# pratyushkumar211/industrial_nnmpc_2021

Hardware: AMD Instinct MI355X
Metric: condensed-QP solves/sec (CDU offline datagen) (higher is better)
Workload: dtype f64; 1 GPU; cdu_offline_data: synthetic CDU-size plant (n=4480 vars, m=8960 box rows, n_aug=284), 100000 sampled x0 per GPU per step, whole sequences u* written out; batch_per_gpu=100000, total_batch=100000, method=auto, parallelism=dp1 (sharded samples, 1 RCCL gather of the first moves pe...

## Files before the change

### industrial_nnmpc_2021_amd/csrc/qp_asm.h

```cpp
#pragma once
#include <hip/hip_runtime.h>
#include <stdint.h>
#include <type_traits>

#if defined(ASM_WG_TU) && ASM_WG_TU >= 0
#define ASM_OWN_KERNELS 0
#else
#define ASM_OWN_KERNELS 1
#endif

namespace nnmpc {

constexpr int ASM_MLDS = 176;
constexpr int ASM_TS = 16 * 17;
enum { ASM_RUN = 0, ASM_DONE = 1, ASM_FALLBACK = 2, ASM_CERT = 3, ASM_WIDE = 4, ASM_INVALID = 5 };
constexpr int ASM_NBIN = 8;
constexpr int ASM_NREG = 6;
constexpr int ASM_NCNT = 40;
constexpr int ASM_CNT_F32 = 16;
constexpr int ASM_NLIST = 2 * ASM_NBIN;
constexpr int ASM_BIG32 = 256;
constexpr int ASM_CNT_BIG64 = 37;
constexpr int ASM_CNT_BIG32 = 36;
constexpr int ASM_BIG32B = 384;
// ... 75 lines not shown
  int* lrank;
  int* ctot;
  int use_f32;
  int W;
  int* rowprob;
  int wrows;
  unsigned char* wmark;
  const double* xhw;
  int tail_gi;
  int use_wg;
  int refine;
  double refine_tol;
  int refine_later;
  int early64;
  int* wflag;
  double* work;
  double* scratch;
  double* u_out;
  int ldu, nout;
  uint32_t* act_out;
  int* status_out;
  int* iters_out;
  int words;
};

__device__ __forceinline__ size_t tri(int i, int j) { return (size_t)i * (i + 1) / 2 + j; }

#if ASM_OWN_KERNELS
__global__ __launch_bounds__(256) void asm_init_k(AsmDev d, int nrows) {
  const int lane = threadIdx.x & 63;
// ... 1262 lines not shown
    d.rounds[p] = rd;
    if (tot > 0 && d.hi[p] < W) d.hi[p] = W;
    const bool refine_next = d.refine_later && m <= ASM_MLDS;
    if (tot == 0 && !grade64 && !(f32_phase && refine_next)) d.prec[p] = 1;
    if (tot > 0 && tot <= d.early64 && f32_phase && !refine_next) d.prec[p] = 1;
    if (settle_wide) d.state[p] = ASM_WIDE;
    else if (settled) {
      d.state[p] = sure ? ASM_CERT : ASM_DONE;
      if (!sure) atomicAdd(&d.counters[ASM_CNT_DONE], 1);
    } else if (rd >= d.max_rounds) d.state[p] = ASM_FALLBACK;
  }
}
#endif

#if ASM_OWN_KERNELS
__global__ __launch_bounds__(256) void asm_wide_k(AsmDev d, int fused_c0) {
  const int lane = threadIdx.x & 63;
  const int w = blockIdx.x * 4 + (threadIdx.x >> 6);
  if (w >= d.wrows) return;
  const int p = d.rowprob[w];
  if (p < 0) return;
  const size_t o = (size_t)p * d.np, orow = (size_t)w * d.np;
  const size_t onar = (size_t)d.row[p] * d.np;
  const int Wp = min(d.W, d.n);
  const bool fused = fused_c0 >= 0;
  const int rend = fused ? min(fused_c0, d.n) : d.n;
  unsigned char* st = d.st + (size_t)p * d.n;
  const int m = d.mg[p];
  const int* idx = d.idxg + (size_t)p * d.max_active;
  int chg = 0;
  double l1 = 0.0, lmin = 1e300;
  for (int i = lane; i < m; i += 64) {
    const double l = d.lam[orow + idx[i]];
    l1 += fabs(l); lmin = fmin(lmin, fabs(l));
  }
  for (int r = lane; r < rend; r += 64) {
    const int k = r % d.nu;
    const double lb = d.lb[(size_t)p * d.nu + k], ub = d.ub[(size_t)p * d.nu + k];
    const int s = st[r];
    double x;
    if (s == 0) {
      x = d.xunc[o + r] - (r < Wp ? d.xh[onar + r] : d.xhw[orow + r]);
      if (x > ub + d.bound_tol) { st[r] = 1; ++chg; }
      else if (x < lb - d.bound_tol) { st[r] = 2; ++chg; }
    } else x = s == 1 ? ub : lb;
    if (r < d.nout) d.u_out[(size_t)p * d.ldu + r] = x;
  }
  if (fused && lane == 0) { chg += d.wflag[p]; d.wflag[p] = 0; }
  double x1 = 0.0;
  for (int k = lane; k < d.ka; k += 64) x1 += fabs(d.x0[(size_t)p * d.ka + k]);
  for (int off = 32; off > 0; off >>= 1) {
    chg += __shfl_xor(chg, off);
    l1 += __shfl_xor(l1, off); x1 += __shfl_xor(x1, off);
    lmin = fmin(lmin, __shfl_xor(lmin, off));
  }
  const int tot = chg;
  const double QI = d.tqmax * x1;
  const double bnd = 2.0 * (d.e1max * x1 + d.e2max * l1) + 1e-14 * (QI + l1) + d.ff_err * (x1 + l1);
  const bool sure = bnd <= d.stat_tol * d.pscale && lmin > bnd;
  if (tot == 0 && !sure) {
    for (int r = lane; r < d.n; r += 64) {
      const int k = r % d.nu, s = st[r];
      double x;
      if (s != 0) x = s == 1 ? d.ub[(size_t)p * d.nu + k] : d.lb[(size_t)p * d.nu + k];
      else if (r < Wp) x = d.xunc[o + r] - d.xh[onar + r];
      else if (!fused) x = d.xunc[o + r] - d.xhw[orow + r];
      else {
        const double* Hc = d.H + r;
        double a0 = 0.0;
        for (int i = 0; i < m; ++i) { const int a = idx[i]; a0 += Hc[(size_t)a * d.np] * d.lam[orow + a]; }
        double xu;
        if (r < d.Wx) xu = d.xunc[o + r];
        else {
          xu = 0.0;
          for (int k2 = 0; k2 < d.ka; ++k2) xu += d.Kunc[(size_t)r * d.ka + k2] * d.x0[(size_t)p * d.ka + k2];
        }
        x = xu - a0;
      }
      d.x[o + r] = x;
    }
  }
  for (int i = lane; i < m; i += 64) d.lam[orow + idx[i]] = 0.0;
  if (lane == 0) {
    d.wmark[p] = 1;
    if (tot == 0) {
      d.state[p] = sure ? ASM_CERT : ASM_DONE;
      if (!sure) atomicAdd(&d.counters[ASM_CNT_DONE], 1);
    } else {
      d.state[p] = d.rounds[p] >= d.max_rounds ? ASM_FALLBACK : ASM_RUN;
      d.ninf_best[p] = 0x7fffffff; d.alpha[p] = ASM_GRACE;
      d.hi[p] = d.n;
    }
  }
}
#endif

constexpr int ASM_FM = 160;
constexpr int ASM_TAIL_GRACE = 2;
constexpr int ASM_TAIL_AREA = ASM_FM * (ASM_FM + 3) / 2 > ASM_TAIL_MB * (ASM_TAIL_MB + 1) / 2 * ASM_TS
                                  ? ASM_FM * (ASM_FM + 3) / 2 : ASM_TAIL_MB * (ASM_TAIL_MB + 1) / 2 * ASM_TS;
constexpr int ASM_TAIL_EXTRA = ASM_FM * (4 + 8 + 8 + 8);
__device__ __forceinline__ int asm_frow(int i) { return i * (i + 3) / 2; }

static_assert(ASM_FM <= 192, "asm_fwd / asm_bwd hold the vector in at most three registers per lane");
template <int NU>
__device__ __forceinline__ void asm_fwd_t(const double* Ld, double* v, int m, int lane) {
  double x[NU], idg[NU], ln[NU];
  const double* rowp[NU];
// ... 446 lines not shown
            --mm;
          }
        }
        if (lane == 0) { s_m = mm; s_fast = ok; }
      }
      __syncthreads();
      m = s_m; fast = s_fast;
    }
    __syncthreads();
  }
  if (tid == 0) { d.state[p] = ASM_FALLBACK; d.rounds[p] = rounds; }
}
#endif

#if ASM_OWN_KERNELS
__global__ __launch_bounds__(256) void asm_certify_k(AsmDev d, double gscale_min) {
  __shared__ int cnt[4];
  __shared__ double gq[4];
  const int p = blockIdx.x, tid = threadIdx.x;
  const int stt = d.state[p];
  if (stt == ASM_INVALID) {
    const double qnan = __longlong_as_double(0x7ff8000000000000ll);
    for (int r = tid; r < d.nout; r += 256) d.u_out[(size_t)p * d.ldu + r] = qnan;
    if (d.act_out) for (int w = tid; w < d.words; w += 256) d.act_out[(size_t)p * d.words + w] = 0u;
    if (tid == 0) {
      if (d.status_out) d.status_out[p] = 2;
      if (d.iters_out) { d.iters_out[2 * p] = 0; d.iters_out[2 * p + 1] = 0; }
    }
    return;
  }
  if (stt != ASM_DONE && stt != ASM_CERT) {
    if (tid == 0 && d.status_out) d.status_out[p] = 3;
    return;
  }
// ... 41 lines not shown
          const int kk = r / d.nu, c = r - kk * d.nu;
          const int bit = kk * 2 * d.nu + (sv == 1 ? c : d.nu + c), w = (bit >> 5) - w0;
          if (w >= 0 && w < nwd) atomicOr(&wb[w], 1u << (bit & 31));
        }
      }
      __syncthreads();
      for (int w = tid; w < nwd; w += 256) d.act_out[(size_t)p * d.words + w0 + w] = wb[w];
      __syncthreads();
    }
  }
  if (tid == 0) {
    if (d.status_out) d.status_out[p] = ok ? 0 : 3;
    if (d.iters_out) { d.iters_out[2 * p] = 0; d.iters_out[2 * p + 1] = 0; }
  }
}
#endif

#if ASM_OWN_KERNELS
__global__ void asm_gather_k(double* x0c, double* lbc, double* ubc, const double* x0, const double* lb,
                             const double* ub, const int* list, int cnt, int n_aug, int nu) {
  const int i = blockIdx.x;
  if (i >= cnt) return;
  const int p = list[i];
  for (int k = threadIdx.x; k < n_aug; k += blockDim.x) x0c[(size_t)i * n_aug + k] = x0[(size_t)p * n_aug + k];
  for (int k = threadIdx.x; k < nu; k += blockDim.x) {
    lbc[(size_t)i * nu + k] = lb[(size_t)p * nu + k];
    ubc[(size_t)i * nu + k] = ub[(size_t)p * nu + k];
  }
}
#endif
// ... 27 lines not shown
```

### industrial_nnmpc_2021_amd/csrc/qp_solver.hip

```cpp
#include <hip/hip_runtime.h>
#include <stdint.h>
#include <stdio.h>
#include <stdarg.h>
#include <string.h>
#include <vector>
#include <algorithm>
#include <cmath>
#include <cstdlib>
#include "../../include/nnmpc.h"
#define ASM_WG_TU (-1)
#include "chol_kernels.h"
#include "gemm_kernels.h"
#include "qp_asm.h"
#include "qp_wide.h"
#include "qp_small.h"
#include "qp_predict.h"
#include "common.h"
static constexpr int ASM_SMALL9_LDS_MAX = 100 * 1024;

using namespace nnmpc;

namespace {

enum { PH_INIT = 0, PH_IPM = 1, PH_POLISH = 2, PH_DONE = 3 };
// ... 588 lines not shown
  double* P64;
  double* tq64;
  float* Kunc32;
  float* pdiag;
  double pscale;
  float* L;
  float* Y;
  float* Dacc;
  unsigned long long* trsv_count;
  QpDev d;
  bool have_inverse;
  double* H64;
  double* Kunc64;
  double *asm_xunc, *asm_x, *asm_lam, *asm_xh, *asm_scratch, *asm_xhw;
  int *asm_rowprob, *asm_wflag;
  unsigned char* asm_wmark;
  unsigned char* asm_st;
  int *asm_state, *asm_rounds, *asm_counters, *asm_biglist, *asm_status, *asm_binlist, *asm_idxg, *asm_mg, *asm_row, *asm_lrank, *asm_ctot;
  unsigned char *asm_prec, *asm_redo, *asm_alpha, *asm_rowk;
  float *asm_lam32, *asm_xh32, *H32;
  int *asm_ninf, *asm_hi, *asm_kblk;
  double tqmax;
  int asm_pool;
  double asm_e1max, asm_e2max;
  struct Far { int W, r, rp; double *U, *Vx, *Vl, *cu; int* kt; double ksum; double efar; };
  std::vector<Far> far;
  std::vector<int> far_missing;
  double p_inf = 0.0;
  double *asm_tnorm = nullptr, *asm_tslack = nullptr;
  struct AsmView {
    double *lam = nullptr, *xh = nullptr, *xhw = nullptr, *tnorm = nullptr, *tslack = nullptr;
// ... 7 lines not shown
  int* pred_cnt = nullptr;
  double* asm_work;
  int seg_max;
  double* x0_64;
  float* x0_32;
  double* q64_all;
  float* uunc_all;
  double *lb_d, *ub_d;
  double* in_stage;
  hipStream_t stream;
  hipStream_t stream2 = nullptr;
  hipStream_t stream3 = nullptr, stream4 = nullptr;
  int asm_tail_budget = 50000;
  hipEvent_t ev_fork = nullptr, ev_join = nullptr, ev_join3 = nullptr, ev_join4 = nullptr;
  hipEvent_t ev_wfork = nullptr, ev_wide = nullptr;
  int* pin_cnt = nullptr;
  int* pin_st = nullptr;
  bool profiling;
  bool gemm_error = false;
  std::vector<hipEvent_t> ev_pool;
  size_t ev_used;
  struct EvRec { int kind; size_t e0, e1; double flops; };
  std::vector<EvRec> ev_recs;
  nnmpc_qp_stats stats;
  std::vector<void*> allocs;
  struct Scratch { void* p = nullptr; size_t cap = 0; };
  enum { SC_U = 0, SC_ACT, SC_ST, SC_IT, SC_GUESS, SC_FB_GUESS, SC_FB_LIST, SC_FB_X0, SC_FB_LB, SC_FB_UB, SC_FB_U, SC_FB_ACT, SC_FB_ST, SC_FB_IT, SC_COUNT };
  Scratch sc[SC_COUNT];
  int ldu, nout;
};
// ... 274 lines not shown
    EvScope es(h, 5, 2.0 * Wx * (double)h->ka * nprob);
    gemm64(h, h->asm_xunc, h->np, h->x0_64, h->ka, h->Kunc64, h->ka, segp, Wx, h->ka);
  }
  AsmDev a;
  a.Kunc = h->Kunc64; a.Wx = Wx; a.winit = winit;
  a.ffU = a.ffVx = a.ffVl = a.ffcu = nullptr; a.ffk = nullptr; a.ffr = a.ffW = 0; a.T = h->asm_xhw; a.tnorm = h->asm_tnorm; a.tslack = h->asm_tslack;
  a.ff_skip = 0; a.ff_err = 0.0; a.ff_efar = 0.0;
  static const bool no_far = getenv("NNMPC_NO_FARFIELD") != nullptr;
  a.n = h->n; a.np = h->np; a.nu = h->nu; a.nseg = nprob;
  a.max_active = h->opts.asm_max_active; a.max_rounds = h->opts.asm_max_rounds;
  a.bound_tol = h->opts.bound_tol; a.stat_tol = 1e-8; a.pscale = h->pscale;
  a.e1max = h->asm_e1max; a.e2max = h->asm_e2max; a.x0 = h->x0_64; a.ka = h->ka;
  a.H = h->H64; a.lb = lb_dev; a.ub = ub_dev; a.xunc = h->asm_xunc; a.q64 = h->q64_all;
  a.x = h->asm_x; a.lam = h->asm_lam; a.xh = h->asm_xh; a.px = h->asm_xh;
  a.st = h->asm_st; a.guess = guess_dev; a.state = h->asm_state; a.rounds = h->asm_rounds; a.counters = h->asm_counters;
  a.biglist = h->asm_biglist; a.binlist = h->asm_binlist; a.idxg = h->asm_idxg; a.mg = h->asm_mg; a.row = h->asm_row; a.tqmax = h->tqmax; a.lrank = h->asm_lrank; a.ctot = h->asm_ctot; a.prec = h->asm_prec; a.redo = h->asm_redo; a.rowk = h->asm_rowk; a.lam32 = h->asm_lam32; a.H32 = h->H32; a.xh32 = h->asm_xh32; a.alpha = h->asm_alpha; a.ninf_best = h->asm_ninf; a.hi = h->asm_hi; a.kblk = h->asm_kblk; a.nkblk = 2 * (h->seg_max / 64 + 2); a.kref = 0; a.use_f32 = h->opts.asm_f32_rounds >= 0; a.xhw = h->asm_xhw; a.rowprob = h->asm_rowprob; a.wrows = 0; a.wmark = h->asm_wmark; a.wflag = h->asm_wflag; a.W = h->np; a.scratch = h->asm_scratch; a.work = h->asm_work;
  a.u_out = u_dev; a.ldu = h->ldu; a.nout = h->nout; a.act_out = act_dev; a.status_out = h->asm_status; a.iters_out = it_dev; a.words = h->words;
  a.nseg = nprob;
  { static const int tgi = getenv("NNMPC_TAIL_GI") ? 1 : 0; a.tail_gi = tgi; }
  { static const int wg = getenv("NNMPC_NO_WG") ? 0 : 1; a.use_wg = wg; }
  { static const int rfn = getenv("NNMPC_REFINE") ? atoi(getenv("NNMPC_REFINE")) : 1; a.refine = 0; a.refine_later = rfn && a.use_f32;
    static const double rtol = getenv("NNMPC_REFINE_TOL") ? atof(getenv("NNMPC_REFINE_TOL")) : ASM_REFINE_TOL; a.refine_tol = rtol; }
  { static const int e64 = getenv("NNMPC_EARLY64") ? atoi(getenv("NNMPC_EARLY64")) : 4; a.early64 = e64; }
  if (!guess_dev) HIPCHK(hipMemsetAsync(h->asm_st, 0, (size_t)nprob * h->n, s));
  a.pred_w = 0; a.pred_f64 = 0;
  double pred_flops_per_it = 0.0;
  {
    static const int env_it = getenv("NNMPC_PRED_ITERS") ? atoi(getenv("NNMPC_PRED_ITERS")) : -1;
    const int iters_req = env_it >= 0 ? (env_it == 0 ? -1 : std::min(env_it, (int)PRED_MAXIT)) : h->opts.asm_predict_iters;
    const int iters = iters_req == 0 ? (int)PRED_MAXIT : iters_req;
    if (iters > 0 && h->pred[0].L > 0.0 && !guess_dev && !small && !tail_only && Wx >= PRED_W) {
// ... 29 lines not shown
      h->stats.asm_predict_launches += 1;
      EvScope es(h, 10, 0.0);
      if (wide) hipLaunchKernelGGL((asm_predict_k<8, 2>), dim3((nprob + 31) / 32), dim3(64 * PRED_NW), (pred_lds_bytes<8, 2>(h->nu)), s, a, pa);
      else if (nu4) hipLaunchKernelGGL((asm_predict_k<4, 4>), dim3((nprob + 63) / 64), dim3(64 * PRED_NW), (pred_lds_bytes<4, 4>(h->nu)), s, a, pa);
      else hipLaunchKernelGGL((asm_predict_k<4, 2, false>), dim3((nprob + 31) / 32), dim3(64 * PRED_NW), (pred_lds_bytes<4, 2>(h->nu)), s, a, pa);
      a.pred_w = W;
      { static const int pf = getenv("NNMPC_PRED_F64") ? atoi(getenv("NNMPC_PRED_F64")) : 0; a.pred_f64 = pf; }
    }
  }
  hipLaunchKernelGGL(asm_init_k, dim3((segp + 3) / 4), dim3(256), 0, s, a, segp);
  const int lds_big = (a.max_active + ASM_TS) * 8;
  int* cnt = h->pin_cnt;
  memset(cnt, 0, 2 * ASM_NCNT * sizeof(int));
  int rounds = 0;
  int kprev = 0;
  HIPCHK(hipMemsetAsync(h->asm_counters, 0, 2 * ASM_NCNT * sizeof(int), s));
  if (small) {
    EvScope es(h, 4, 0.0);
    static const int g0 = getenv("NNMPC_SMALL_GRACE") ? atoi(getenv("NNMPC_SMALL_GRACE")) : ASM_SM_GRACE;
    hipLaunchKernelGGL((asm_small_k<2, 3, 4>), dim3(nprob), dim3(64), asm_small_lds_bytes(2, h->n, h->nu), s, a, a.max_rounds, g0);
    hipLaunchKernelGGL((asm_small_k<7, 1, 8>), dim3(nprob), dim3(64), asm_small_lds_bytes(7, h->n, h->nu), s, a, a.max_rounds, g0);
    if (asm_small_lds_bytes(9, h->n, h->nu) <= ASM_SMALL9_LDS_MAX)
      hipLaunchKernelGGL((asm_small_k<9, 1, 8>), dim3(nprob), dim3(64), asm_small_lds_bytes(9, h->n, h->nu), s, a, a.max_rounds, g0);
    h->stats.asm_rounds += 1;
    h->stats.asm_small_passes += 1;
    static const bool trace = getenv("NNMPC_TRACE_ROUNDS") != nullptr;
    if (trace) {
      std::vector<int> rd(nprob), mg(nprob), stt(nprob);
      HIPCHK(stream_sync(s));
      hipMemcpy(rd.data(), h->asm_rounds, nprob * sizeof(int), hipMemcpyDeviceToHost);
      hipMemcpy(mg.data(), h->asm_mg, nprob * sizeof(int), hipMemcpyDeviceToHost);
// ... 33 lines not shown
      std::vector<int> rd(nprob), mg(nprob);
      hipMemcpy(rd.data(), h->asm_rounds, nprob * sizeof(int), hipMemcpyDeviceToHost);
      hipMemcpy(mg.data(), h->asm_mg, nprob * sizeof(int), hipMemcpyDeviceToHost);
      long sum = 0, sm = 0; int mx = 0, mm = 0;
      for (int i = 0; i < nprob; ++i) { sum += rd[i]; mx = std::max(mx, rd[i]); sm += mg[i]; mm = std::max(mm, mg[i]); }
      fprintf(stderr, "asm tail only: %d problems, iterations mean %.2f max %d, active bounds mean %.1f max %d\n", nprob, (double)sum / nprob, mx, (double)sm / nprob, mm);
    }
  }
  auto set_view = [&](AsmDev& d, int v) {
    const nnmpc_qp::AsmView& V = h->view[v];
    d.lam = V.lam; d.xh = V.xh; d.xhw = V.xhw; d.T = V.xhw; d.tnorm = V.tnorm; d.tslack = V.tslack; d.lam32 = V.lam32; d.xh32 = V.xh32;
    d.rowprob = V.rowprob; d.kblk = V.kblk; d.counters = V.counters;
  };
  const char* env_ovl = getenv("NNMPC_OVERLAP");
  const bool overlap_on = h->opts.asm_overlap >= 0 && h->view[1].rows > 0 && !(env_ovl && atoi(env_ovl) == 0);
  int vW[2] = {h->np, h->np}, vrows[2] = {0, 0};
  int pend = -1;
  bool tail_ran[2] = {false, false};
  struct WideStat { bool open; int view, far_rp, skip, cols; double far_ksum; } wst = {false, 0, 0, 0, 0, 0.0}, wnext = wst;
  int fft_prev[2] = {0, 0};
  auto account = [&](const int* c) {
    if (!wst.open) return;
    wst.open = false;
    if (!h->profiling) return;
    const double nw = c[ASM_CNT_WIDE + 1], ksum = c[ASM_CNT_WKSUM];
    if (wst.far_rp) {
      const int fft = h->pin_cnt[wst.view * ASM_NCNT + ASM_CNT_FFTILES];
      const double chunks = fft - fft_prev[wst.view];
      fft_prev[wst.view] = fft;
      h->stats.asm_gemm_flops += 2.0 * wst.far_rp * (ksum + nw * h->ka) +
// ... 36 lines not shown
        HIPCHK(hipStreamWaitEvent(ps, h->ev_wfork, 0));
      }
      ap.ff_err = 0.0; ap.ff_efar = 0.0; ap.ff_skip = 0;
      int far_rp = 0;
      double far_ksum = 0.0;
      {
        EvScope es(h, 5, 0.0, ps);
        if (ff) {
          ap.ffU = ff->U; ap.ffVx = ff->Vx; ap.ffVl = ff->Vl; ap.ffcu = ff->cu; ap.ffk = ff->kt; ap.ffr = ff->rp; ap.ffW = ff->W;
          ap.ff_err = h->p_inf * ff->efar; ap.ff_efar = ff->efar;
          ap.ff_skip = h->nout <= c0 && h->nout < h->n;
          far_rp = ff->rp; far_ksum = ff->ksum;
          h->stats.asm_far_passes += 1;
          hipLaunchKernelGGL(asm_wide_t_k, dim3(g64_grid(ntm, ff->rp / 128)), dim3(256), G64_LDS, ps, ap, ntm, ff->rp / 128);
          if (ap.ff_skip) hipLaunchKernelGGL(asm_wide_tnorm_k, dim3((ntm * 128 + 3) / 4), dim3(256), 0, ps, ap, ntm);
          hipLaunchKernelGGL(asm_wide_gemm_k<WIDE_FAR>, dim3(g64_grid(ntm, ntn)), dim3(256), G64_LDS, ps, ap, c0, ntm, ntn);
        } else if (fused_c0 >= 0 && lazy) {
          hipLaunchKernelGGL(asm_wide_gemm_k<WIDE_LAZY>, dim3(g64_grid(ntm, ntn)), dim3(256), G64_LDS, s, ap, c0, ntm, ntn);
        } else if (fused_c0 >= 0) {
          hipLaunchKernelGGL(asm_wide_gemm_k<WIDE_XUNC>, dim3(g64_grid(ntm, ntn)), dim3(256), G64_LDS, s, ap, c0, ntm, ntn);
        } else {
          gemm64(h, h->view[pv].xhw + c0, h->np, h->view[pv].lam, h->np, h->H64 + (size_t)c0 * h->np, h->np, ((prev_rows + 127) / 128) * 128,
                 h->np - c0, h->np, nullptr, 0, h->view[pv].kblk, nullptr, true);
        }
      }
      wnext.view = pv; wnext.far_rp = far_rp; wnext.far_ksum = far_ksum; wnext.skip = ap.ff_skip; wnext.cols = h->np - c0; wnext.open = true;
      if (ovl) {
        HIPCHK(hipEventRecord(h->ev_wide, ps));
        inflight = true;
      } else {
        EvScope es(h, 6, 0.0);
        hipLaunchKernelGGL(asm_wide_k, dim3((prev_rows + 3) / 4), dim3(256), 0, s, ap, fused_c0);
        wst = wnext;
      }
      pend = -1; vrows[pv] = 0;
    }
    auto finish_pass = [&]() -> int {
      HIPCHK(hipStreamWaitEvent(s, h->ev_wide, 0));
      EvScope es(h, 6, 0.0);
      hipLaunchKernelGGL(asm_wide_k, dim3((ap.wrows + 3) / 4), dim3(256), 0, s, ap, fused_c0);
      wst = wnext;
      inflight = false;
      return 0;
    };
    if (!a.pred_w) a.refine_later = 0;
    a.refine = a.refine_later && rounds >= 1;
    a.kref = kprev;
    int rv = inflight ? 1 - pv : 0;
    int n64 = 0, n32 = 0, nrun = 0;
    for (;;) {
      set_view(a, rv);
      cnt = h->pin_cnt + rv * ASM_NCNT;
      {
        EvScope es(h, 6, 0.0);
        hipLaunchKernelGGL(asm_count_k, dim3((nprob + 3) / 4), dim3(256), 0, s, a);
// ... 158 lines not shown
    }
  }
  if (rounds >= 2 * a.max_rounds + 2) {
    HIPCHK(hipMemcpyAsync(h->pin_cnt, h->asm_counters, 2 * ASM_NCNT * sizeof(int), hipMemcpyDeviceToHost, s));
    HIPCHK(stream_sync(s));
  }
  if (h->gemm_error) { h->gemm_error = false; return NNMPC_EINVAL; }
  set_view(a, 0);
  cnt = h->pin_cnt;
  auto ndone = [&]() { return h->pin_cnt[ASM_CNT_DONE] + h->pin_cnt[ASM_NCNT + ASM_CNT_DONE]; };
  if (!defer_cnt) h->stats.asm_full_checks += ndone();
  if (defer_cnt || ndone() > 0) {
    gemm64(h, h->q64_all, h->np, h->x0_64, h->ka, h->tq64, h->ka, segp, h->np, h->ka, h->asm_state, ASM_DONE);
    gemm64(h, h->asm_xh, h->np, h->asm_x, h->np, h->P64, h->np, segp, h->np, h->np, h->asm_state, ASM_DONE);
  }
  hipLaunchKernelGGL(asm_certify_k, dim3(nprob), dim3(256), 0, s, a, h->pscale);
  int* st = h->pin_st;
  HIPCHK(hipMemcpyAsync(st, h->asm_status, (size_t)nprob * sizeof(int), hipMemcpyDeviceToHost, s));
  int* pin_its = h->pin_cnt + 2 * ASM_NCNT;
  if (h->profiling && pred_flops_per_it > 0.0) HIPCHK(hipMemcpyAsync(pin_its, h->pred_cnt + 1, 4, hipMemcpyDeviceToHost, s));
  if (defer_cnt) HIPCHK(hipMemcpyAsync(h->pin_cnt, h->asm_counters, 2 * ASM_NCNT * sizeof(int), hipMemcpyDeviceToHost, s));
  HIPCHK(stream_sync(s));
  if (defer_cnt) h->stats.asm_full_checks += ndone();
  if (h->profiling && pred_flops_per_it > 0.0) h->stats.asm_predict_flops += pred_flops_per_it * (double)*pin_its;
  HIPCHK(hipGetLastError());
  std::vector<int> fb;
  int ninvalid = 0;
  for (int p = 0; p < nprob; ++p) { if (st[p] == 3) fb.push_back(p); else if (st[p] != 0) ++ninvalid; }
  h->stats.asm_solved += nprob - (int64_t)fb.size() - ninvalid;
  if (st_dev) HIPCHK(hipMemcpyAsync(st_dev, h->asm_status, (size_t)nprob * sizeof(int), hipMemcpyDeviceToDevice, s));
  if (fb.empty()) { h->stats.problems += nprob; return 0; }
// ... 86 lines not shown
  h->n = n; h->nu = nu; h->n_aug = n_aug;
  h->NB = o.nb;
  h->np = ((n + h->NB - 1) / h->NB) * h->NB;
  h->T = h->np / h->NB;
  h->tiles = h->T * (h->T + 1) / 2;
  h->ka = ((n_aug + 31) / 32) * 32;
  h->slots = ((o.max_batch + 127) / 128) * 128;
  h->words = (2 * n + 31) / 32;
  h->have_kunc = Kunc != nullptr;
  if ((size_t)(h->np + 5 * h->NB) * 4 > 96 * 1024) { set_error("n too large for the LDS-resident solve vector"); delete h; return NNMPC_EINVAL; }
  if (hipStreamCreate(&h->stream) != hipSuccess) { set_error("hipStreamCreate failed"); delete h; return NNMPC_EHIP; }
  if (hipStreamCreate(&h->stream2) != hipSuccess || hipStreamCreate(&h->stream3) != hipSuccess || hipStreamCreate(&h->stream4) != hipSuccess ||
      hipEventCreateWithFlags(&h->ev_fork, hipEventDisableTiming) != hipSuccess ||
      hipEventCreateWithFlags(&h->ev_join3, hipEventDisableTiming) != hipSuccess || hipEventCreateWithFlags(&h->ev_join4, hipEventDisableTiming) != hipSuccess ||
      hipEventCreateWithFlags(&h->ev_join, hipEventDisableTiming) != hipSuccess ||
      hipEventCreateWithFlags(&h->ev_wfork, hipEventDisableTiming) != hipSuccess || hipEventCreateWithFlags(&h->ev_wide, hipEventDisableTiming) != hipSuccess) {
    set_error("hipStreamCreate / hipEventCreate failed"); nnmpc_qp_destroy(h); return NNMPC_EHIP;
  }
  {
    hipError_t e = hipSuccess;
    if (e == hipSuccess) e = hipFuncSetAttribute((const void*)asm_lambda_reg_k, hipFuncAttributeMaxDynamicSharedMemorySize, ASM_REG_LDS);
    if (e == hipSuccess) e = hipFuncSetAttribute((const void*)asm_lambda_reg2_k, hipFuncAttributeMaxDynamicSharedMemorySize, ASM_REG2_LDS);
    if (e == hipSuccess) e = hipFuncSetAttribute((const void*)asm_lambda_reg32_k, hipFuncAttributeMaxDynamicSharedMemorySize, ASM_REG32_LDS);
    if (e == hipSuccess) e = hipFuncSetAttribute((const void*)asm_tail_k, hipFuncAttributeMaxDynamicSharedMemorySize, 150 * 1024);
    if (e == hipSuccess) e = hipFuncSetAttribute((const void*)asm_lambda_reg32b_k, hipFuncAttributeMaxDynamicSharedMemorySize, ASM_REG32B_LDS);
    if (e == hipSuccess) e = hipFuncSetAttribute((const void*)asm_lambda_tile32_k, hipFuncAttributeMaxDynamicSharedMemorySize, ASM_TILE32_LDS);
    if (e == hipSuccess) e = hipFuncSetAttribute((const void*)gemm_nt_f64_t128_k, hipFuncAttributeMaxDynamicSharedMemorySize, G64_LDS);
    if (e == hipSuccess) e = hipFuncSetAttribute((const void*)asm_wide_gemm_k<WIDE_XUNC>, hipFuncAttributeMaxDynamicSharedMemorySize, G64_LDS);
    if (e == hipSuccess) e = hipFuncSetAttribute((const void*)asm_wide_gemm_k<WIDE_LAZY>, hipFuncAttributeMaxDynamicSharedMemorySize, G64_LDS);
    if (e == hipSuccess) e = hipFuncSetAttribute((const void*)asm_wide_gemm_k<WIDE_FAR>, hipFuncAttributeMaxDynamicSharedMemorySize, G64_LDS);
    if (e == hipSuccess) e = hipFuncSetAttribute((const void*)asm_wide_t_k, hipFuncAttributeMaxDynamicSharedMemorySize, G64_LDS);
// ... 29 lines not shown
    cap = std::min<long long>(cap, 1 << 20);
    h->seg_max = (int)((cap / 128) * 128);
  }
  const size_t G = h->seg_max;
  A_(h->x0_64, G * ka); A_(h->x0_32, G * ka);
  A_(h->q64_all, G * np); A_(h->uunc_all, G * np);
  A_(h->lb_d, G * nu); A_(h->ub_d, G * nu);
  A_(h->in_stage, G * n_aug);
  if (!rc && hipHostMalloc((void**)&h->pin_cnt, (2 * ASM_NCNT + 4) * sizeof(int)) != hipSuccess) { set_error("nnmpc_qp_create: hipHostMalloc failed"); rc = NNMPC_EHIP; }
  if (!rc && hipHostMalloc((void**)&h->pin_st, G * sizeof(int)) != hipSuccess) { set_error("nnmpc_qp_create: hipHostMalloc failed"); rc = NNMPC_EHIP; }
  A_(d.lb64, (size_t)S * nu); A_(d.ub64, (size_t)S * nu);
  A_(d.slot_prob, S); A_(d.age, S); A_(d.next_prob, 1);
  h->asm_pool = h->seg_max >= 4096 ? (getenv("NNMPC_TAIL_MAX") && atoi(getenv("NNMPC_TAIL_MAX")) > 1024 ? 2048 : 1024) : 256;
  A_(h->H64, (size_t)np * np); A_(h->Kunc64, (size_t)np * ka); A_(h->H32, (size_t)np * np);
  A_(h->asm_xunc, G * np); A_(h->asm_x, G * np); A_(h->asm_lam, G * np); A_(h->asm_xh, G * np);
  A_(h->asm_xhw, (G + 256) * np); A_(h->asm_rowprob, G + 256); A_(h->asm_wflag, G); A_(h->asm_wmark, G);
  A_(h->asm_tnorm, G + 128 * (ASM_NKG + 1)); A_(h->asm_tslack, G + 128 * (ASM_NKG + 1));
  A_(h->asm_st, G * n); A_(h->asm_state, G); A_(h->asm_rounds, G); A_(h->asm_counters, 2 * ASM_NCNT);
  A_(h->asm_biglist, G); A_(h->asm_status, G); A_(h->asm_binlist, (size_t)(ASM_NLIST + 4) * G);
  A_(h->asm_idxg, G * o.asm_max_active); A_(h->asm_mg, G); A_(h->asm_row, G); A_(h->asm_lrank, G); A_(h->asm_ctot, ((G + 1023) / 1024) * ASM_NSCAN); A_(h->asm_prec, G); A_(h->asm_redo, G); A_(h->asm_rowk, G); A_(h->asm_lam32, G * np); A_(h->asm_xh32, G * np); A_(h->asm_alpha, G); A_(h->asm_ninf, G); A_(h->asm_hi, G); A_(h->asm_kblk, 2 * (G / 64 + 2)); A_(h->asm_work, 3 * G);
  A_(h->asm_scratch, (size_t)h->asm_pool * ((size_t)(o.asm_max_active / 16) * (o.asm_max_active / 16 + 1) / 2 * ASM_TS));
  {
    nnmpc_qp::AsmView& v0 = h->view[0];
    v0.lam = h->asm_lam; v0.xh = h->asm_xh; v0.xhw = h->asm_xhw; v0.tnorm = h->asm_tnorm; v0.tslack = h->asm_tslack;
    v0.lam32 = h->asm_lam32; v0.xh32 = h->asm_xh32; v0.rowprob = h->asm_rowprob; v0.kblk = h->asm_kblk; v0.counters = h->asm_counters;
    v0.rows = (int)G;
    long long R = std::max<long long>(1024, ((long long)G / 32 + 127) / 128 * 128);
    if (const char* e = getenv("NNMPC_OVERLAP_ROWS")) R = std::max(0, atoi(e) / 128 * 128);
    R = std::min<long long>(R, (long long)G);
    if (o.asm_overlap >= 0 && R > 0) {
      nnmpc_qp::AsmView& v1 = h->view[1];
      const size_t Rr = (size_t)R;
      A_(v1.lam, Rr * np); A_(v1.xh, Rr * np); A_(v1.xhw, (Rr + 256) * np); A_(v1.lam32, Rr * np); A_(v1.xh32, Rr * np);
// ... 69 lines not shown
}

int nnmpc_qp_destroy(nnmpc_qp* h) {
  if (!h) return NNMPC_OK;
  hipDeviceSynchronize();
  for (void* p : h->allocs) hipFree(p);
  for (auto& g : h->far) { hipFree(g.U); hipFree(g.Vx); hipFree(g.Vl); hipFree(g.cu); hipFree(g.kt); }
  for (auto& sc : h->sc) if (sc.p) hipFree(sc.p);
  for (hipEvent_t e : h->ev_pool) hipEventDestroy(e);
  if (h->ev_fork) hipEventDestroy(h->ev_fork);
  if (h->ev_join) hipEventDestroy(h->ev_join);
  if (h->ev_join3) hipEventDestroy(h->ev_join3);
  if (h->ev_join4) hipEventDestroy(h->ev_join4);
  if (h->ev_wfork) hipEventDestroy(h->ev_wfork);
  if (h->ev_wide) hipEventDestroy(h->ev_wide);
  if (h->pin_cnt) hipHostFree(h->pin_cnt);
  if (h->pin_st) hipHostFree(h->pin_st);
  if (h->stream2) hipStreamDestroy(h->stream2);
  if (h->stream3) hipStreamDestroy(h->stream3);
  if (h->stream4) hipStreamDestroy(h->stream4);
  if (h->stream) hipStreamDestroy(h->stream);
  delete h;
  return NNMPC_OK;
}

int nnmpc_qp_set_inverse(nnmpc_qp* h, const double* Hinv, const double* Kunc) {
  if (!h || !Hinv || !Kunc) { set_error("nnmpc_qp_set_inverse: bad arguments"); return NNMPC_EINVAL; }
  HIPCHK(hipSetDevice(h->device));
  const int n = h->n, np = h->np, ka = h->ka, n_aug = h->n_aug;
  if ((uint64_t)np * np * 8 >= (1ull << 32)) {
// ... 300 lines not shown
```

Baseline: 7.635 million solves/s.

## Split wide-pass finish to overlap with far GEMM; wave-per-problem certify kernel

The wide-pass epilogue is split in two. A pre-kernel does the bound check and certificate test as soon as the lambda-dependent work is recorded, overlapping the far-side wide GEMM on the side stream. A decision kernel then finishes after the GEMM completes. Certification now runs one wave per problem for certified, invalid and other-state cases, compacting DONE problems into a list that a block-per-problem kernel processes. The goal is to hide wide-pass latency and cut idle blocks in certify, at the cost of extra launches, events and an atomic list counter.

```diff
diff --git a/industrial_nnmpc_2021_amd/csrc/qp_asm.h b/industrial_nnmpc_2021_amd/csrc/qp_asm.h
--- a/industrial_nnmpc_2021_amd/csrc/qp_asm.h
+++ b/industrial_nnmpc_2021_amd/csrc/qp_asm.h
@@ -113,6 +113,8 @@
   int refine_later;
   int early64;
   int* wflag;
+  unsigned char* wpre;
+  int* certn;
   double* work;
   double* scratch;
   double* u_out;
@@ -1405,50 +1407,12 @@
 #endif
 
 #if ASM_OWN_KERNELS
-__global__ __launch_bounds__(256) void asm_wide_k(AsmDev d, int fused_c0) {
-  const int lane = threadIdx.x & 63;
-  const int w = blockIdx.x * 4 + (threadIdx.x >> 6);
-  if (w >= d.wrows) return;
-  const int p = d.rowprob[w];
-  if (p < 0) return;
-  const size_t o = (size_t)p * d.np, orow = (size_t)w * d.np;
-  const size_t onar = (size_t)d.row[p] * d.np;
+__device__ __forceinline__ void asm_wide_finish(const AsmDev& d, int p, int w, int lane, bool fused, int tot, bool sure, bool zero_lam) {
+  const size_t o = (size_t)p * d.np, orow = (size_t)w * d.np, onar = (size_t)d.row[p] * d.np;
   const int Wp = min(d.W, d.n);
-  const bool fused = fused_c0 >= 0;
-  const int rend = fused ? min(fused_c0, d.n) : d.n;
-  unsigned char* st = d.st + (size_t)p * d.n;
+  const unsigned char* st = d.st + (size_t)p * d.n;
   const int m = d.mg[p];
   const int* idx = d.idxg + (size_t)p * d.max_active;
-  int chg = 0;
-  double l1 = 0.0, lmin = 1e300;
-  for (int i = lane; i < m; i += 64) {
-    const double l = d.lam[orow + idx[i]];
-    l1 += fabs(l); lmin = fmin(lmin, fabs(l));
-  }
-  for (int r = lane; r < rend; r += 64) {
-    const int k = r % d.nu;
-    const double lb = d.lb[(size_t)p * d.nu + k], ub = d.ub[(size_t)p * d.nu + k];
-    const int s = st[r];
-    double x;
-    if (s == 0) {
-      x = d.xunc[o + r] - (r < Wp ? d.xh[onar + r] : d.xhw[orow + r]);
-      if (x > ub + d.bound_tol) { st[r] = 1; ++chg; }
-      else if (x < lb - d.bound_tol) { st[r] = 2; ++chg; }
-    } else x = s == 1 ? ub : lb;
-    if (r < d.nout) d.u_out[(size_t)p * d.ldu + r] = x;
-  }
-  if (fused && lane == 0) { chg += d.wflag[p]; d.wflag[p] = 0; }
-  double x1 = 0.0;
-  for (int k = lane; k < d.ka; k += 64) x1 += fabs(d.x0[(size_t)p * d.ka + k]);
-  for (int off = 32; off > 0; off >>= 1) {
-    chg += __shfl_xor(chg, off);
-    l1 += __shfl_xor(l1, off); x1 += __shfl_xor(x1, off);
-    lmin = fmin(lmin, __shfl_xor(lmin, off));
-  }
-  const int tot = chg;
-  const double QI = d.tqmax * x1;
-  const double bnd = 2.0 * (d.e1max * x1 + d.e2max * l1) + 1e-14 * (QI + l1) + d.ff_err * (x1 + l1);
-  const bool sure = bnd <= d.stat_tol * d.pscale && lmin > bnd;
   if (tot == 0 && !sure) {
     for (int r = lane; r < d.n; r += 64) {
       const int k = r % d.nu, s = st[r];
@@ -1471,7 +1435,7 @@
       d.x[o + r] = x;
     }
   }
-  for (int i = lane; i < m; i += 64) d.lam[orow + idx[i]] = 0.0;
+  if (zero_lam) for (int i = lane; i < m; i += 64) d.lam[orow + idx[i]] = 0.0;
   if (lane == 0) {
     d.wmark[p] = 1;
     if (tot == 0) {
@@ -1483,6 +1447,90 @@
       d.hi[p] = d.n;
     }
   }
+}
+#endif
+
+#if ASM_OWN_KERNELS
+__device__ __forceinline__ int asm_wide_window(const AsmDev& d, int p, int w, int lane, int rend, bool& sure) {
+  const size_t o = (size_t)p * d.np, orow = (size_t)w * d.np;
+  const size_t onar = (size_t)d.row[p] * d.np;
+  const int Wp = min(d.W, d.n);
+  unsigned char* st = d.st + (size_t)p * d.n;
+  const int m = d.mg[p];
+  const int* idx = d.idxg + (size_t)p * d.max_active;
+  int chg = 0;
+  double l1 = 0.0, lmin = 1e300;
+  for (int i = lane; i < m; i += 64) {
+    const double l = d.lam[orow + idx[i]];
+    l1 += fabs(l); lmin = fmin(lmin, fabs(l));
+  }
+  for (int r = lane; r < rend; r += 64) {
+    const int k = r % d.nu;
+    const double lb = d.lb[(size_t)p * d.nu + k], ub = d.ub[(size_t)p * d.nu + k];
+    const int s = st[r];
+    double x;
+    if (s == 0) {
+      x = d.xunc[o + r] - (r < Wp ? d.xh[onar + r] : d.xhw[orow + r]);
+      if (x > ub + d.bound_tol) { st[r] = 1; ++chg; }
+      else if (x < lb - d.bound_tol) { st[r] = 2; ++chg; }
+    } else x = s == 1 ? ub : lb;
+    if (r < d.nout) d.u_out[(size_t)p * d.ldu + r] = x;
+  }
+  double x1 = 0.0;
+  for (int k = lane; k < d.ka; k += 64) x1 += fabs(d.x0[(size_t)p * d.ka + k]);
+  for (int off = 32; off > 0; off >>= 1) {
+    chg += __shfl_xor(chg, off);
+    l1 += __shfl_xor(l1, off); x1 += __shfl_xor(x1, off);
+    lmin = fmin(lmin, __shfl_xor(lmin, off));
+  }
+  const double QI = d.tqmax * x1;
+  const double bnd = 2.0 * (d.e1max * x1 + d.e2max * l1) + 1e-14 * (QI + l1) + d.ff_err * (x1 + l1);
+  sure = bnd <= d.stat_tol * d.pscale && lmin > bnd;
+  return chg;
+}
+#endif
+
+#if ASM_OWN_KERNELS
+__global__ __launch_bounds__(256) void asm_wide_k(AsmDev d, int fused_c0) {
+  const int lane = threadIdx.x & 63;
+  const int w = blockIdx.x * 4 + (threadIdx.x >> 6);
+  if (w >= d.wrows) return;
+  const int p = d.rowprob[w];
+  if (p < 0) return;
+  const bool fused = fused_c0 >= 0;
+  bool sure;
+  int tot = asm_wide_window(d, p, w, lane, fused ? min(fused_c0, d.n) : d.n, sure);
+  if (fused) { tot += d.wflag[p]; if (lane == 0) d.wflag[p] = 0; }
+  asm_wide_finish(d, p, w, lane, fused, tot, sure, true);
+}
+
+__global__ __launch_bounds__(256) void asm_wide_pre_k(AsmDev d, int fused_c0) {
+  const int lane = threadIdx.x & 63;
+  const int w = blockIdx.x * 4 + (threadIdx.x >> 6);
+  if (w >= d.wrows) return;
+  const int p = d.rowprob[w];
+  if (p < 0) return;
+  bool sure;
+  const int chg = asm_wide_window(d, p, w, lane, min(fused_c0, d.n), sure);
+  if (sure) {
+    const size_t orow = (size_t)w * d.np;
+    const int m = d.mg[p];
+    const int* idx = d.idxg + (size_t)p * d.max_active;
+    for (int i = lane; i < m; i += 64) d.lam[orow + idx[i]] = 0.0;
+  }
+  if (lane == 0) d.wpre[p] = (unsigned char)((sure ? 1 : 0) | (chg > 0 ? 2 : 0));
+}
+__global__ __launch_bounds__(256) void asm_wide_dec_k(AsmDev d) {
+  const int lane = threadIdx.x & 63;
+  const int w = blockIdx.x * 4 + (threadIdx.x >> 6);
+  if (w >= d.wrows) return;
+  const int p = d.rowprob[w];
+  if (p < 0) return;
+  const int pre = d.wpre[p];
+  const bool sure = (pre & 1) != 0;
+  const int tot = (pre >> 1) + d.wflag[p];
+  if (lane == 0) d.wflag[p] = 0;
+  asm_wide_finish(d, p, w, lane, true, tot, sure, !sure);
 }
 #endif
 
@@ -1959,10 +2007,10 @@
 #endif
 
 #if ASM_OWN_KERNELS
-__global__ __launch_bounds__(256) void asm_certify_k(AsmDev d, double gscale_min) {
+__device__ __forceinline__ void asm_certify_one(const AsmDev& d, double gscale_min, int p) {
   __shared__ int cnt[4];
   __shared__ double gq[4];
-  const int p = blockIdx.x, tid = threadIdx.x;
+  const int tid = threadIdx.x;
   const int stt = d.state[p];
   if (stt == ASM_INVALID) {
     const double qnan = __longlong_as_double(0x7ff8000000000000ll);
@@ -2034,6 +2082,106 @@
     if (d.iters_out) { d.iters_out[2 * p] = 0; d.iters_out[2 * p + 1] = 0; }
   }
 }
+__global__ __launch_bounds__(256) void asm_certify_k(AsmDev d, double gscale_min) { asm_certify_one(d, gscale_min, blockIdx.x); }
+
+__global__ __launch_bounds__(256) void asm_certify_list_k(AsmDev d, double gscale_min) {
+  const int nl = *d.certn;
+  for (int i = blockIdx.x; i < nl; i += gridDim.x) {
+    asm_certify_one(d, gscale_min, d.biglist[i]);
+    __syncthreads();
+  }
+}
+
+__global__ __launch_bounds__(256) void asm_certify_wave_k(AsmDev d, double gscale_min) {
+  __shared__ uint32_t wbs[4][256];
+  const int lane = threadIdx.x & 63, wv = threadIdx.x >> 6;
+  const int p = blockIdx.x * 4 + wv;
+  if (p >= d.nseg) return;
+  const int stt = d.state[p];
+  if (stt == ASM_DONE) {
+    if (lane == 0) d.biglist[atomicAdd(d.certn, 1)] = p;
+    return;
+  }
+  if (stt == ASM_INVALID) {
+    const double qnan = __longlong_as_double(0x7ff8000000000000ll);
+    for (int r = lane; r < d.nout; r += 64) d.u_out[(size_t)p * d.ldu + r] = qnan;
+    if (d.act_out) for (int w = lane; w < d.words; w += 64) d.act_out[(size_t)p * d.words + w] = 0u;
+    if (lane == 0) {
+      if (d.status_out) d.status_out[p] = 2;
+      if (d.iters_out) { d.iters_out[2 * p] = 0; d.iters_out[2 * p + 1] = 0; }
+    }
+    return;
+  }
+  if (stt != ASM_CERT) {
+    if (lane == 0 && d.status_out) d.status_out[p] = 3;
+    return;
+  }
+  const int ok = 0.0 <= d.stat_tol * fmax(gscale_min, 0.0);
+  if (d.act_out) {
+    uint32_t* ao = d.act_out + (size_t)p * d.words;
+    const unsigned char* st = d.st + (size_t)p * d.n;
+    const int nu = d.nu;
+    const int rlim = min((min(d.hi[p], d.n) + nu - 1) / nu * nu, d.n);
+    const bool whole = d.n % nu == 0;
+    if (whole && nu < 32 && 32 % nu == 0) {
+      const uint32_t msk = (1u << nu) - 1u;
+      for (int r0 = 0; r0 < rlim; r0 += 64) {
+        const int r = r0 + lane;
+        const int sv = r < rlim ? st[r] : 0;
+        const unsigned long long U = __ballot(sv == 1), L = __ballot(sv == 2);
+        const int w = (r0 >> 4) + lane;
+        if (lane < 4 && w < d.words) {
+          const uint32_t u16 = (uint32_t)(U >> (16 * lane)) & 0xffffu, l16 = (uint32_t)(L >> (16 * lane)) & 0xffffu;
+          uint32_t word = 0u;
+          for (int g = 0; g * nu < 16; ++g)
+            word |= (((u16 >> (g * nu)) & msk) << (2 * g * nu)) | (((l16 >> (g * nu)) & msk) << (2 * g * nu + nu));
+          ao[w] = word;
+        }
+      }
+      for (int w = min(d.words, (rlim + 63) / 64 * 4) + lane; w < d.words; w += 64) ao[w] = 0u;
+    } else if (whole && nu % 32 == 0) {
+      const int cps = nu / 32;
+      for (int r0 = 0; r0 < rlim; r0 += 64) {
+        const int r = r0 + lane;
+        const int sv = r < rlim ? st[r] : 0;
+        const unsigned long long U = __ballot(sv == 1), L = __ballot(sv == 2);
+        const int j = (r0 >> 5) + (lane >> 1);
+        if (lane < 4 && 32 * j < rlim) {
+          const int kk = j / cps, cj = j - kk * cps;
+          ao[kk * 2 * cps + (lane & 1) * cps + cj] = (uint32_t)(((lane & 1) ? L : U) >> (32 * (lane >> 1)));
+        }
+      }
+      for (int w = rlim / nu * 2 * cps + lane; w < d.words; w += 64) ao[w] = 0u;
+    } else {
+      uint32_t* wb = wbs[wv];
+      for (int w0 = 0; w0 < d.words; w0 += 256) {
+        const int nwd = min(256, d.words - w0);
+        const int k0 = (32 * w0) / (2 * nu), k1 = min(rlim / nu + (rlim % nu != 0), (32 * (w0 + nwd) + 2 * nu - 1) / (2 * nu));
+        if (k0 * nu >= rlim) {
+          for (int w = lane; w < nwd; w += 64) ao[w0 + w] = 0u;
+          continue;
+        }
+        for (int w = lane; w < nwd; w += 64) wb[w] = 0u;
+        ASM_FENCE();
+        for (int r = k0 * nu + lane; r < min(k1 * nu, rlim); r += 64) {
+          const int sv = st[r];
+          if (sv) {
+            const int kk = r / nu, c = r - kk * nu;
+            const int bit = kk * 2 * nu + (sv == 1 ? c : nu + c), w = (bit >> 5) - w0;
+            if (w >= 0 && w < nwd) atomicOr(&wb[w], 1u << (bit & 31));
+          }
+        }
+        ASM_FENCE();
+        for (int w = lane; w < nwd; w += 64) ao[w0 + w] = wb[w];
+        ASM_FENCE();
+      }
+    }
+  }
+  if (lane == 0) {
+    if (d.status_out) d.status_out[p] = ok ? 0 : 3;
+    if (d.iters_out) { d.iters_out[2 * p] = 0; d.iters_out[2 * p + 1] = 0; }
+  }
+}
 #endif
 
 #if ASM_OWN_KERNELS
diff --git a/industrial_nnmpc_2021_amd/csrc/qp_solver.hip b/industrial_nnmpc_2021_amd/csrc/qp_solver.hip
--- a/industrial_nnmpc_2021_amd/csrc/qp_solver.hip
+++ b/industrial_nnmpc_2021_amd/csrc/qp_solver.hip
@@ -626,7 +626,7 @@
   double* Kunc64;
   double *asm_xunc, *asm_x, *asm_lam, *asm_xh, *asm_scratch, *asm_xhw;
   int *asm_rowprob, *asm_wflag;
-  unsigned char* asm_wmark;
+  unsigned char *asm_wmark, *asm_wpre;
   unsigned char* asm_st;
   int *asm_state, *asm_rounds, *asm_counters, *asm_biglist, *asm_status, *asm_binlist, *asm_idxg, *asm_mg, *asm_row, *asm_lrank, *asm_ctot;
   unsigned char *asm_prec, *asm_redo, *asm_alpha, *asm_rowk;
@@ -664,6 +664,7 @@
   int asm_tail_budget = 50000;
   hipEvent_t ev_fork = nullptr, ev_join = nullptr, ev_join3 = nullptr, ev_join4 = nullptr;
   hipEvent_t ev_wfork = nullptr, ev_wide = nullptr;
+  hipEvent_t ev_wlam = nullptr;
   int* pin_cnt = nullptr;
   int* pin_st = nullptr;
   bool profiling;
@@ -968,7 +969,7 @@
   a.H = h->H64; a.lb = lb_dev; a.ub = ub_dev; a.xunc = h->asm_xunc; a.q64 = h->q64_all;
   a.x = h->asm_x; a.lam = h->asm_lam; a.xh = h->asm_xh; a.px = h->asm_xh;
   a.st = h->asm_st; a.guess = guess_dev; a.state = h->asm_state; a.rounds = h->asm_rounds; a.counters = h->asm_counters;
-  a.biglist = h->asm_biglist; a.binlist = h->asm_binlist; a.idxg = h->asm_idxg; a.mg = h->asm_mg; a.row = h->asm_row; a.tqmax = h->tqmax; a.lrank = h->asm_lrank; a.ctot = h->asm_ctot; a.prec = h->asm_prec; a.redo = h->asm_redo; a.rowk = h->asm_rowk; a.lam32 = h->asm_lam32; a.H32 = h->H32; a.xh32 = h->asm_xh32; a.alpha = h->asm_alpha; a.ninf_best = h->asm_ninf; a.hi = h->asm_hi; a.kblk = h->asm_kblk; a.nkblk = 2 * (h->seg_max / 64 + 2); a.kref = 0; a.use_f32 = h->opts.asm_f32_rounds >= 0; a.xhw = h->asm_xhw; a.rowprob = h->asm_rowprob; a.wrows = 0; a.wmark = h->asm_wmark; a.wflag = h->asm_wflag; a.W = h->np; a.scratch = h->asm_scratch; a.work = h->asm_work;
+  a.biglist = h->asm_biglist; a.binlist = h->asm_binlist; a.idxg = h->asm_idxg; a.mg = h->asm_mg; a.row = h->asm_row; a.tqmax = h->tqmax; a.lrank = h->asm_lrank; a.ctot = h->asm_ctot; a.prec = h->asm_prec; a.redo = h->asm_redo; a.rowk = h->asm_rowk; a.lam32 = h->asm_lam32; a.H32 = h->H32; a.xh32 = h->asm_xh32; a.alpha = h->asm_alpha; a.ninf_best = h->asm_ninf; a.hi = h->asm_hi; a.kblk = h->asm_kblk; a.nkblk = 2 * (h->seg_max / 64 + 2); a.kref = 0; a.use_f32 = h->opts.asm_f32_rounds >= 0; a.xhw = h->asm_xhw; a.rowprob = h->asm_rowprob; a.wrows = 0; a.wmark = h->asm_wmark; a.wpre = h->asm_wpre; a.certn = h->asm_counters + 2 * ASM_NCNT; a.wflag = h->asm_wflag; a.W = h->np; a.scratch = h->asm_scratch; a.work = h->asm_work;
   a.u_out = u_dev; a.ldu = h->ldu; a.nout = h->nout; a.act_out = act_dev; a.status_out = h->asm_status; a.iters_out = it_dev; a.words = h->words;
   a.nseg = nprob;
   { static const int tgi = getenv("NNMPC_TAIL_GI") ? 1 : 0; a.tail_gi = tgi; }
@@ -1028,7 +1029,7 @@
   memset(cnt, 0, 2 * ASM_NCNT * sizeof(int));
   int rounds = 0;
   int kprev = 0;
-  HIPCHK(hipMemsetAsync(h->asm_counters, 0, 2 * ASM_NCNT * sizeof(int), s));
+  HIPCHK(hipMemsetAsync(h->asm_counters, 0, (2 * ASM_NCNT + 1) * sizeof(int), s));
   if (small) {
     EvScope es(h, 4, 0.0);
     static const int g0 = getenv("NNMPC_SMALL_GRACE") ? atoi(getenv("NNMPC_SMALL_GRACE")) : ASM_SM_GRACE;
@@ -1092,6 +1093,8 @@
   };
   const char* env_ovl = getenv("NNMPC_OVERLAP");
   const bool overlap_on = h->opts.asm_overlap >= 0 && h->view[1].rows > 0 && !(env_ovl && atoi(env_ovl) == 0);
+  const char* env_split = getenv("NNMPC_WIDE_SPLIT");
+  const bool wide_split = !(env_split && atoi(env_split) == 0);
   int vW[2] = {h->np, h->np}, vrows[2] = {0, 0};
   int pend = -1;
   bool tail_ran[2] = {false, false};
@@ -1158,6 +1161,7 @@
           h->stats.asm_far_passes += 1;
           hipLaunchKernelGGL(asm_wide_t_k, dim3(g64_grid(ntm, ff->rp / 128)), dim3(256), G64_LDS, ps, ap, ntm, ff->rp / 128);
           if (ap.ff_skip) hipLaunchKernelGGL(asm_wide_tnorm_k, dim3((ntm * 128 + 3) / 4), dim3(256), 0, ps, ap, ntm);
+          if (ovl && wide_split) HIPCHK(hipEventRecord(h->ev_wlam, ps));
           hipLaunchKernelGGL(asm_wide_gemm_k<WIDE_FAR>, dim3(g64_grid(ntm, ntn)), dim3(256), G64_LDS, ps, ap, c0, ntm, ntn);
         } else if (fused_c0 >= 0 && lazy) {
           hipLaunchKernelGGL(asm_wide_gemm_k<WIDE_LAZY>, dim3(g64_grid(ntm, ntn)), dim3(256), G64_LDS, s, ap, c0, ntm, ntn);
@@ -1180,9 +1184,17 @@
       pend = -1; vrows[pv] = 0;
     }
     auto finish_pass = [&]() -> int {
-      HIPCHK(hipStreamWaitEvent(s, h->ev_wide, 0));
-      EvScope es(h, 6, 0.0);
-      hipLaunchKernelGGL(asm_wide_k, dim3((ap.wrows + 3) / 4), dim3(256), 0, s, ap, fused_c0);
+      if (wide_split) {
+        HIPCHK(hipStreamWaitEvent(s, h->ev_wlam, 0));
+        { EvScope es(h, 6, 0.0); hipLaunchKernelGGL(asm_wide_pre_k, dim3((ap.wrows + 3) / 4), dim3(256), 0, s, ap, fused_c0); }
+        HIPCHK(hipStreamWaitEvent(s, h->ev_wide, 0));
+        EvScope es(h, 6, 0.0);
+        hipLaunchKernelGGL(asm_wide_dec_k, dim3((ap.wrows + 3) / 4), dim3(256), 0, s, ap);
+      } else {
+        HIPCHK(hipStreamWaitEvent(s, h->ev_wide, 0));
+        EvScope es(h, 6, 0.0);
+        hipLaunchKernelGGL(asm_wide_k, dim3((ap.wrows + 3) / 4), dim3(256), 0, s, ap, fused_c0);
+      }
       wst = wnext;
       inflight = false;
       return 0;
@@ -1371,7 +1383,14 @@
     gemm64(h, h->q64_all, h->np, h->x0_64, h->ka, h->tq64, h->ka, segp, h->np, h->ka, h->asm_state, ASM_DONE);
     gemm64(h, h->asm_xh, h->np, h->asm_x, h->np, h->P64, h->np, segp, h->np, h->np, h->asm_state, ASM_DONE);
   }
-  hipLaunchKernelGGL(asm_certify_k, dim3(nprob), dim3(256), 0, s, a, h->pscale);
+  const char* env_cw = getenv("NNMPC_CERT_WAVE");
+  if (defer_cnt || (env_cw && atoi(env_cw) == 0)) {
+    hipLaunchKernelGGL(asm_certify_k, dim3(nprob), dim3(256), 0, s, a, h->pscale);
+  } else {
+    hipLaunchKernelGGL(asm_certify_wave_k, dim3((nprob + 3) / 4), dim3(256), 0, s, a, h->pscale);
+    const int nlist = std::min(ndone(), nprob);
+    if (nlist > 0) hipLaunchKernelGGL(asm_certify_list_k, dim3(nlist), dim3(256), 0, s, a, h->pscale);
+  }
   int* st = h->pin_st;
   HIPCHK(hipMemcpyAsync(st, h->asm_status, (size_t)nprob * sizeof(int), hipMemcpyDeviceToHost, s));
   int* pin_its = h->pin_cnt + 2 * ASM_NCNT;
@@ -1488,7 +1507,8 @@
       hipEventCreateWithFlags(&h->ev_fork, hipEventDisableTiming) != hipSuccess ||
       hipEventCreateWithFlags(&h->ev_join3, hipEventDisableTiming) != hipSuccess || hipEventCreateWithFlags(&h->ev_join4, hipEventDisableTiming) != hipSuccess ||
       hipEventCreateWithFlags(&h->ev_join, hipEventDisableTiming) != hipSuccess ||
-      hipEventCreateWithFlags(&h->ev_wfork, hipEventDisableTiming) != hipSuccess || hipEventCreateWithFlags(&h->ev_wide, hipEventDisableTiming) != hipSuccess) {
+      hipEventCreateWithFlags(&h->ev_wfork, hipEventDisableTiming) != hipSuccess || hipEventCreateWithFlags(&h->ev_wide, hipEventDisableTiming) != hipSuccess ||
+      hipEventCreateWithFlags(&h->ev_wlam, hipEventDisableTiming) != hipSuccess) {
     set_error("hipStreamCreate / hipEventCreate failed"); nnmpc_qp_destroy(h); return NNMPC_EHIP;
   }
   {
@@ -1548,9 +1568,9 @@
   h->asm_pool = h->seg_max >= 4096 ? (getenv("NNMPC_TAIL_MAX") && atoi(getenv("NNMPC_TAIL_MAX")) > 1024 ? 2048 : 1024) : 256;
   A_(h->H64, (size_t)np * np); A_(h->Kunc64, (size_t)np * ka); A_(h->H32, (size_t)np * np);
   A_(h->asm_xunc, G * np); A_(h->asm_x, G * np); A_(h->asm_lam, G * np); A_(h->asm_xh, G * np);
-  A_(h->asm_xhw, (G + 256) * np); A_(h->asm_rowprob, G + 256); A_(h->asm_wflag, G); A_(h->asm_wmark, G);
+  A_(h->asm_xhw, (G + 256) * np); A_(h->asm_rowprob, G + 256); A_(h->asm_wflag, G); A_(h->asm_wmark, G); A_(h->asm_wpre, G);
   A_(h->asm_tnorm, G + 128 * (ASM_NKG + 1)); A_(h->asm_tslack, G + 128 * (ASM_NKG + 1));
-  A_(h->asm_st, G * n); A_(h->asm_state, G); A_(h->asm_rounds, G); A_(h->asm_counters, 2 * ASM_NCNT);
+  A_(h->asm_st, G * n); A_(h->asm_state, G); A_(h->asm_rounds, G); A_(h->asm_counters, 2 * ASM_NCNT + 1);
   A_(h->asm_biglist, G); A_(h->asm_status, G); A_(h->asm_binlist, (size_t)(ASM_NLIST + 4) * G);
   A_(h->asm_idxg, G * o.asm_max_active); A_(h->asm_mg, G); A_(h->asm_row, G); A_(h->asm_lrank, G); A_(h->asm_ctot, ((G + 1023) / 1024) * ASM_NSCAN); A_(h->asm_prec, G); A_(h->asm_redo, G); A_(h->asm_rowk, G); A_(h->asm_lam32, G * np); A_(h->asm_xh32, G * np); A_(h->asm_alpha, G); A_(h->asm_ninf, G); A_(h->asm_hi, G); A_(h->asm_kblk, 2 * (G / 64 + 2)); A_(h->asm_work, 3 * G);
   A_(h->asm_scratch, (size_t)h->asm_pool * ((size_t)(o.asm_max_active / 16) * (o.asm_max_active / 16 + 1) / 2 * ASM_TS));
@@ -1650,6 +1670,7 @@
   if (h->ev_join4) hipEventDestroy(h->ev_join4);
   if (h->ev_wfork) hipEventDestroy(h->ev_wfork);
   if (h->ev_wide) hipEventDestroy(h->ev_wide);
+  if (h->ev_wlam) hipEventDestroy(h->ev_wlam);
   if (h->pin_cnt) hipHostFree(h->pin_cnt);
   if (h->pin_st) hipHostFree(h->pin_st);
   if (h->stream2) hipStreamDestroy(h->stream2);
```

Result: no change. 7.684 million solves/s, median of 6 (+0.6%).
